# ratan-lab/indelMINER

Hardware: AMD Instinct MI355X
Metric: reads/sec through split-read realign+cluster; VCF diff-clean vs reference (higher is better)
Workload: dtype u8/int32; 1 GPU; BASELINE configs[1]: synthetic 1.0 Mb contig per GPU, 100 bp PE reads at 30x, seeded 1-50 bp indels every ~2 kb, BWA-like S/I/D emission; -k 6 -g 0 -s 1000 -n 10 -q 10; pipeline_depth=4, hip_graph=True, parallelism=contig-sharded x1

## Files before the change

### indelminer_amd/csrc/im_capi.hip

```cpp

#include "im_device.hpp"

#include <stdarg.h>
#include <stdio.h>
#include <stdlib.h>
#include <string.h>

#include <algorithm>
#include <vector>
#include <unordered_map>
#include <mutex>
#include <atomic>

struct ContigArray {
    int32_t* data = nullptr;
    int32_t* sums = nullptr;
    int64_t cap = 0, len = -1;
};

struct GenomeArray {
    int32_t* data = nullptr;
    int32_t* sums = nullptr;
    int32_t flank = 0, min_mapq = 0;
};
// ... 16 lines not shown
    size_t pin_bytes = 0;
    hipStream_t copy_stream = nullptr, back_stream = nullptr;
    hipEvent_t ev_in[2] = {nullptr, nullptr}, ev_k[2] = {nullptr, nullptr}, ev_out[2] = {nullptr, nullptr};
    ContigArray depth, span, pair;
    ContigArray clip_r, clip_l;
    std::vector<int64_t> h_asc_off;
    std::vector<int32_t> h_len;
    int64_t ref_total = 0;
    GenomeArray all_depth, all_span, all_pair;
    GenomeArray all_clip_r, all_clip_l;
    im::TailTable tail = {nullptr, nullptr, 0};
    int32_t tail_min_clip = 0, tail_min_mapq = 0;
    im::LinkTable link = {nullptr, nullptr, 0};
    int32_t link_min_mapq = 0;
    uint32_t* med_scratch = nullptr;
    int32_t med_slots = 0;
    bool med_dirty = false;
    bool support_count_attr = false;
    std::mutex gb_mu;
    std::unordered_map<void*, int32_t> gb_layout;
    std::unordered_map<void*, std::pair<int32_t, int32_t>> fg_layout;
    std::vector<int64_t> h_sums_off;
    void* rg_blob = nullptr;
    im::RgTable rg = {nullptr, 0, 0};
    std::mutex any_mu;
    int32_t* any_list = nullptr; int32_t any_list_cap = 0;
    int32_t* any_counters = nullptr;
    int32_t* any_arena = nullptr; size_t any_arena_bytes = 0;
};

namespace {

char g_err[512] = "";

void set_err(im_ctx* ctx, const char* fmt, ...)
{
    va_list ap;
    va_start(ap, fmt);
    char* dst = ctx ? ctx->err : g_err;
    vsnprintf(dst, 512, fmt, ap);
    va_end(ap);
}

#define HIP_TRY(ctx, expr)                                                              \
    do {                                                                                \
        hipError_t e_ = (expr);                                                         \
        if (e_ != hipSuccess) {                                                         \
// ... 241 lines not shown
    ctx->h_sums_off = sums_off;
    HIP_TRY(ctx, hipMalloc((void**)&g.data, (size_t)ctx->ref_total * sizeof(int32_t)));
    if (scanned) HIP_TRY(ctx, hipMalloc((void**)&g.sums, (size_t)(ints + 1) * sizeof(int32_t)));
    HIP_TRY(ctx, hipMemsetAsync(g.data, 0, (size_t)ctx->ref_total * sizeof(int32_t), ctx->stream));
    if (scanned) HIP_TRY(ctx, hipMemsetAsync(g.sums, 0, (size_t)(ints + 1) * sizeof(int32_t), ctx->stream));
    HIP_TRY(ctx, hipStreamSynchronize(ctx->stream));
    if (flank) { g.flank = *flank; g.min_mapq = min_mapq; }
    return IM_OK;
}

int scan_genome_array(im_ctx* ctx, GenomeArray im_ctx::*which, int32_t tid, void* stream)
{
    if (!ctx || !(ctx->*which).data || tid < 0 || tid >= ctx->n_contigs) return IM_E_ARG;
    const GenomeArray& g = ctx->*which;
    HIP_TRY(ctx, hipSetDevice(ctx->device));
    HIP_TRY(ctx, im::launch_depth_scan_tiled(g.data + ctx->h_asc_off[tid], (int64_t)ctx->h_len[tid] + 1, g.sums + ctx->h_sums_off[tid], (hipStream_t)stream));
    return IM_OK;
}

int reset_genome_array(im_ctx* ctx, GenomeArray im_ctx::*which, int32_t tid, void* stream)
{
    if (!ctx || !(ctx->*which).data || tid < 0 || tid >= ctx->n_contigs) return IM_E_ARG;
    HIP_TRY(ctx, hipSetDevice(ctx->device));
    HIP_TRY(ctx, hipMemsetAsync((ctx->*which).data + ctx->h_asc_off[tid], 0, ((size_t)ctx->h_len[tid] + 1) * sizeof(int32_t), (hipStream_t)stream));
    return IM_OK;
}

int query_genome_array(im_ctx* ctx, GenomeArray im_ctx::*which, int32_t tid, int32_t n, const int32_t* beg, const int32_t* end, Reduce what,
                       uint32_t* out, uint32_t* max_out, const ArgMaxSide* argmax = nullptr)
{
    if (!ctx || n < 0 || !(ctx->*which).data || tid < 0 || tid >= ctx->n_contigs) return IM_E_ARG;
    if (n == 0) return IM_OK;
    if (!beg || !end || !out) return IM_E_ARG;
    const GenomeArray& g = ctx->*which;
    const int32_t* sums = g.sums ? g.sums + ctx->h_sums_off[tid] : nullptr;
    return query_array(ctx, n, beg, end, g.data + ctx->h_asc_off[tid], sums, ctx->h_len[tid], what, out, max_out, argmax);
}

im::RefDev ref_dev(const im_ctx* ctx)
{
    im::RefDev ref;
    ref.ascii = ctx->ref_ascii; ref.pk = reinterpret_cast<const uint8_t*>(ctx->ref_pk);
    ref.asc_off = ctx->d_asc_off; ref.pk_off = ctx->d_pk_off; ref.len = ctx->d_len; ref.n_contigs = ctx->n_contigs;
    return ref;
}

}
// ... 212 lines not shown
        bin_start[b] = e;
        for (int32_t i = n - 1; i >= 0; i--) {
            if (bin[i] != b) continue;
            name_off[e] = (int32_t)names.size();
            name_len[e] = (int32_t)strlen(names_in[i]);
            rmax[e] = range_max[i];
            names.insert(names.end(), names_in[i], names_in[i] + name_len[e] + 1);
            e++;
        }
    }
    bin_start[16] = e;
    std::vector<uint8_t> host((size_t)4 * (20 + 3 * (size_t)m) + names.size() + 8, 0);
    memcpy(host.data(), bin_start.data(), 80);
    memcpy(host.data() + 80, name_off.data(), 4 * (size_t)m);
    memcpy(host.data() + 80 + 4 * (size_t)m, name_len.data(), 4 * (size_t)m);
    memcpy(host.data() + 80 + 8 * (size_t)m, rmax.data(), 4 * (size_t)m);
    if (!names.empty()) memcpy(host.data() + 80 + 12 * (size_t)m, names.data(), names.size());
    const size_t total = (host.size() + 3) / 4 * 4;
    host.resize(total, 0);
    if (ctx->rg_blob) { HIP_TRY(ctx, hipFree(ctx->rg_blob)); ctx->rg_blob = nullptr; }
    HIP_TRY(ctx, hipMalloc(&ctx->rg_blob, total + 256));
    HIP_TRY(ctx, hipMemcpy(ctx->rg_blob, host.data(), total, hipMemcpyHostToDevice));
    ctx->rg.blob = (const uint8_t*)ctx->rg_blob; ctx->rg.n = n; ctx->rg.bytes = (int32_t)total;
    return IM_OK;
}

size_t im_dev_triage_scratch_bytes(int32_t n_records) { return im::triage_scratch_bytes(n_records); }

int im_dev_triage_scratch_init(im_ctx* ctx, int32_t n_records, void* scratch, size_t scratch_bytes, void* stream)
{
    if (!ctx || !scratch || scratch_bytes < im::triage_scratch_bytes(n_records)) return IM_E_ARG;
    HIP_TRY(ctx, hipSetDevice(ctx->device));
    size_t zb = 0;
    const size_t off = im::triage_scratch_zero_offset(n_records, &zb);
    HIP_TRY(ctx, hipMemsetAsync((char*)scratch + off, 0, zb, (hipStream_t)stream));
    return IM_OK;
}

int im_dev_triage(im_ctx* ctx, const im_triage_params* tp, const im_dev_records* recs, const im_dev_cands* out,
                  void* scratch, size_t scratch_bytes, void* stream)
{
    if (!ctx || !tp || !recs || !out) return IM_E_ARG;
    if (!ctx->ref_ascii) { set_err(ctx, "im_set_reference has not been called"); return IM_E_ARG; }
    if (!ctx->rg_blob) { set_err(ctx, "im_set_insert_ranges has not been called"); return IM_E_ARG; }
    if (recs->n < 0 || !out->counters || !out->cand_rec) { set_err(ctx, "bad triage arguments"); return IM_E_ARG; }
    if (scratch_bytes < im::triage_scratch_bytes(recs->n)) { set_err(ctx, "triage scratch too small"); return IM_E_ARG; }
// ... 1297 lines not shown
```

### indelminer_amd/csrc/im_depth.hip

```cpp

#include "im_device.hpp"

namespace im {
namespace {

constexpr int kScanBlock = 256;
constexpr int kScanItems = 8;
constexpr int kScanSub = kScanBlock * kScanItems;
constexpr int kScanSubs = kScanTile / kScanSub;
constexpr int kScanWaves = kScanBlock / 64;
static_assert(kScanTile == kScanSub * kScanSubs, "im_device.hpp names the tile for the queries");
constexpr int kScanGroup = 32;
constexpr int kOffItems = 4;

__global__ __launch_bounds__(256) void depth_scatter_kernel(int32_t n_seg, const int32_t* __restrict__ start, const int32_t* __restrict__ len,
                                                           int64_t clen, int64_t lo, int64_t hi, int32_t* __restrict__ diff)
{
    for (int64_t i = blockIdx.x * (int64_t)blockDim.x + threadIdx.x; i < n_seg; i += (int64_t)gridDim.x * blockDim.x) {
        int64_t a = start[i], b = (int64_t)start[i] + len[i];
        if (a < 0) a = 0;
        if (b > clen) b = clen;
        if (a + lo >= b - hi) continue;
        atomicAdd(&diff[a + lo], 1);
        atomicAdd(&diff[b - hi], -1);
// ... 239 lines not shown
        }
        if (lane == 63) {
#pragma unroll
            for (int s = 0; s < kMedSegs; s++) wsum[s * kMedWaves + wave] = x[s];
        }
        __syncthreads();
        const uint32_t want = (uint32_t)((b - a + 1) / 2);
        uint32_t pre = 0;
#pragma unroll
        for (int s = 0; s < kMedSegs; s++) {
            uint32_t front = 0;
#pragma unroll
            for (int k = 0; k < kMedWaves; k++) { if (k == wave) front = pre; pre += wsum[s * kMedWaves + k]; }
            uint32_t acc = front + x[s] - run[s];
            if (acc < want && want <= acc + run[s]) {
                int e = 0;
                for (; e < 3; e++) { acc += c[s][e]; if (acc >= want) break; }
                out[q] = (uint32_t)((s * kMedBlock + tid) * 4 + e);
            }
        }
    }
}

}

int64_t depth_sums_ints(int64_t clen) { const int64_t t = (clen + 1 + kScanTile - 1) / kScanTile; return t + 1 + (t + kScanGroup - 1) / kScanGroup; }

hipError_t launch_depth_scan_tiled(int32_t* depth, int64_t n, int32_t* sums, hipStream_t stream)
{
    if (n <= 0) return hipSuccess;
    const int64_t tiles = (n + kScanTile - 1) / kScanTile;
    hipLaunchKernelGGL(depth_scan_tiled_kernel, dim3((int)tiles), dim3(kScanBlock), 0, stream, depth, n, sums, (int32_t)tiles);
    return hipGetLastError();
}

hipError_t launch_depth_build(int64_t clen, int32_t n_seg, const int32_t* seg_start, const int32_t* seg_len, int32_t lo, int32_t hi,
                              int32_t* data, int32_t* sums, hipStream_t stream)
{
    const int64_t n = clen + 1;
    hipError_t e = hipMemsetAsync(data, 0, (size_t)n * sizeof(int32_t), stream);
    if (e == hipSuccess) e = hipMemsetAsync(sums, 0, (size_t)depth_sums_ints(clen) * sizeof(int32_t), stream);
    if (e != hipSuccess) return e;
    if (n_seg > 0) {
        int64_t b = ((int64_t)n_seg + 255) / 256;
        if (b > 4096) b = 4096;
        hipLaunchKernelGGL(depth_scatter_kernel, dim3((int)b), dim3(256), 0, stream, n_seg, seg_start, seg_len, clen, (int64_t)lo, (int64_t)hi, data);
// ... 38 lines not shown
```

### indelminer_amd/csrc/im_device.hpp

```cpp
#pragma once

#include <hip/hip_runtime.h>
#include <stdint.h>

#include "indelminer_amd.h"

namespace im {

struct RefDev {
    const uint8_t*  ascii;
    const uint8_t*  pk;
    const int64_t*  asc_off;
    const int64_t*  pk_off;
    const int32_t*  len;
    int32_t         n_contigs;
};

constexpr int kShortRead = 255;
constexpr int kMaxWaveGaps = 60;

struct RealignArgs {
    RefDev      ref;
    im_dev_batch batch;
    im_params   P;
    int32_t     keep_slots;
    const int32_t* n_dev;
    int32_t     first;
};

struct RgTable {
    const uint8_t* blob;
    int32_t n;
    int32_t bytes;
};

size_t triage_scratch_bytes(int32_t n_records);
size_t triage_scratch_zero_offset(int32_t n_records, size_t* bytes);
hipError_t launch_triage(const RefDev& ref, const RgTable& rg, int32_t* depth_diff, const im_triage_params& tp,
                         const im_dev_records& recs, const im_dev_cands& out, void* scratch, hipStream_t stream);

hipError_t launch_flush_cut(const int32_t* cls, const int32_t* b1, const int32_t* b2, int32_t* consumed,
                            int32_t a0, int32_t a1, int32_t b0, int32_t b1_end, int32_t marker, int32_t flush_id,
                            uint64_t* cut_word, const int32_t* cand_rec, const int32_t* n_cand_dev, int32_t cand_cap, hipStream_t stream);
hipError_t launch_flush_seq(const im_flush_desc* desc, int32_t n_fl, const int32_t* cls, const int32_t* b1, const int32_t* b2,
                            int32_t* consumed, const int32_t* cand_rec, const int32_t* n_cand_dev, int32_t cand_cap, int32_t pe_base,
                            int32_t pe_count, hipStream_t stream);
size_t groupby_scratch_bytes(int32_t n_slots);
hipError_t launch_groupby_init(int32_t n_slots, void* scratch, hipStream_t stream);
hipError_t launch_groupby(int32_t n_layout, int32_t n_slots, const int32_t* n_cand_dev, const int32_t* cls, const int32_t* b1, const int32_t* b2, const int32_t* consumed,
                          int32_t tie_desc, int32_t* order, int32_t* cl_key, int32_t* cl_first, int32_t* cl_count,
                          int32_t* counts, void* scratch, hipStream_t stream);
size_t flushgroup_scratch_bytes(int32_t n_slots, int32_t n_fl_cap);
hipError_t launch_flushgroup_init(int32_t n_slots, int32_t n_fl_cap, void* scratch, hipStream_t stream);
hipError_t launch_flush_groupby(int32_t n_slots_layout, int32_t n_fl_layout, const im_flush_desc* desc, int32_t n_fl,
                                const int32_t* cls, const int32_t* b1, const int32_t* b2, int32_t* consumed,
                                const int32_t* cand_rec, const int32_t* n_cand_dev, int32_t cand_cap, int32_t pe_base, int32_t pe_count,
                                int32_t tie_desc, int32_t* order, int32_t* cl_key, int32_t* cl_first, int32_t* cl_count, int32_t* counts,
                                void* scratch, hipStream_t stream);

constexpr int kScanTile = 8192;
int64_t depth_sums_ints(int64_t clen);
hipError_t launch_depth_scan_tiled(int32_t* depth, int64_t n, int32_t* sums, hipStream_t stream);
hipError_t launch_depth_build(int64_t clen, int32_t n_seg, const int32_t* seg_start, const int32_t* seg_len, int32_t lo, int32_t hi,
                              int32_t* data, int32_t* sums, hipStream_t stream);
hipError_t launch_depth_query_tiled(int32_t nq, const int32_t* beg, const int32_t* end, const int32_t* depth, const int32_t* sums,
                                    int64_t clen, uint32_t* out, uint32_t* out_max, hipStream_t stream);
int32_t depth_median_slabs(int32_t beg, int32_t end, int64_t clen);
size_t depth_median_scratch_bytes(int32_t slots);
hipError_t launch_depth_median(int32_t nq, int32_t items, const int32_t* beg, const int32_t* end, const int32_t* first, const int32_t* slot,
                               const int32_t* data, const int32_t* sums, int64_t clen, uint32_t* scratch, int32_t slots, int32_t max_blocks,
                               uint32_t* out, hipStream_t stream);

hipError_t launch_pack_reference(const uint8_t* ascii, uint64_t* pk, int64_t n_bases_padded,
                                 hipStream_t stream);
hipError_t launch_realign(const RealignArgs& a, int n_cu, hipStream_t stream);
hipError_t launch_realign_long(const RealignArgs& a, int n_cu, hipStream_t stream);

hipError_t launch_realign_any_pick(const RealignArgs& a, int all, int32_t* list, int32_t* counters, hipStream_t stream);
size_t realign_any_arena_bytes(int32_t max_read, int32_t max_window, uint32_t numgaps, int32_t lane_shift, int32_t n_waves);
hipError_t launch_realign_any(const RealignArgs& a, const int32_t* list, int32_t* counters, int32_t* arena,
                              int32_t max_read, int32_t max_window, int32_t lane_shift, int32_t n_waves, hipStream_t stream);

hipError_t launch_compact_results(const im_read_result* res, int32_t n_cap, const int32_t* n_dev, int32_t* status, int32_t* slot,
                                  im_read_result* compact, int32_t* count, int n_cu, hipStream_t stream);

// ... 68 lines not shown
```

### indelminer_amd/csrc/im_triage.hip

```cpp

#include "im_device.hpp"
#include "im_rg.hpp"

namespace im {
namespace {

constexpr int kTriBlock = 256;
constexpr int kTriGroup = 32;
constexpr int kTriGroupsMax = 2048;

__device__ __forceinline__ uint32_t ld_u16(const uint8_t* p) { uint16_t v; __builtin_memcpy(&v, p, 2); return v; }


__device__ __forceinline__ uint32_t cigar_word(const RecView& r, uint32_t k)
{
    return k == 0u ? r.cig[0] : k == 1u ? r.cig[1] : k == 2u ? r.cig[2] : k == 3u ? r.cig[3] : ld_u32(r.p + r.o_cigar + 4u * k);
}

__device__ __forceinline__ int32_t aux_int(const RecView& r, const AuxWin& w, uint32_t o)
{
    const uint32_t type = rec_byte(r, w, o);
    if (o + 1u >= r.len) return 0;
    const uint32_t b0 = rec_byte(r, w, o + 1);
    switch (type) {
// ... 171 lines not shown
}

struct TriageArgs {
    im_dev_records recs;
    im_dev_cands out;
    im_triage_params tp;
    RefDev ref;
    RgTable rg;
    int32_t* depth_diff;
    uint32_t* info;
    int32_t* rmax;
    uint2* blk;
    uint32_t* blocks_done;
    uint32_t* grp_done;
    unsigned long long* grp;
    uint2* grp_base;
    int32_t group_size;
    uint32_t* seq_at;
    int32_t* chunk_base;
};

__device__ __forceinline__ uint32_t padded4(int32_t l) { return ((uint32_t)l + 3u) & ~3u; }

constexpr int kDepthWin = 4096;

__global__ __launch_bounds__(kTriBlock, 6) void triage_classify_kernel(TriageArgs A)
{
    __shared__ uint32_t s_cnt[kTriBlock / 64], s_bytes[kTriBlock / 64], s_counted[kTriBlock / 64], s_err[kTriBlock / 64];
    __shared__ uint32_t s_aux[kTriBlock][kAuxWin / 4];
    __shared__ uint32_t s_rg[kRgLds / 4];
    __shared__ int32_t s_generic[2];
    __shared__ int32_t s_dd[kDepthWin];
    __shared__ int32_t s_wpos[kTriBlock / 64], s_wtid[kTriBlock / 64];
    __shared__ uint32_t s_fb[kTriBlock];
    const int t = threadIdx.x, lane = t & 63, wave = t >> 6;
    const int64_t i = (int64_t)blockIdx.x * kTriBlock + t;
    if (A.depth_diff) {
        int4* z = reinterpret_cast<int4*>(s_dd);
#pragma unroll
        for (int k = 0; k < kDepthWin / 4 / kTriBlock; k++) z[t + k * kTriBlock] = make_int4(0, 0, 0, 0);
    }

    RecView r; r.ok = false; r.l_seq = 0; r.flag = 0; r.n_cigar = 0; r.tid = -1; r.pos = 0; r.o_cigar = 0; r.o_seq = 0; r.p = A.recs.raw; r.len = 0; r.o_aux = 0;
    s_fb[t] = 0xFFFFFFFFu;
    if (i < A.recs.n) r = view_record(A.recs.raw, A.recs.rec_off[i], A.recs.rec_off[i + 1]);
    const uint32_t sw_lim = reaches_new_readaln(r) ? (uint32_t)r.l_seq : 0u;
    const uint32_t sw_so = sw_lim ? (uint32_t)(r.p - A.recs.raw) + r.o_seq : 0u;
    BaseSweep S;
    sweep_issue(S, A.recs.raw, sw_so, sw_lim, lane);
    if (r.ok) {
#pragma unroll
        for (int k = 0; k < 4; k++) r.cig[k] = ld_u32(r.p + r.o_cigar + 4u * k);
        const uint32_t aux_bytes = r.len - r.o_aux;
#pragma unroll
        for (int k = 0; k < kAuxWin / 4; k++) if (4u * k < aux_bytes) s_aux[t][k] = ld_u32(r.p + r.o_aux + 4u * k);
    }
    sweep_finish(S, A.recs.raw, sw_so, sw_lim, s_fb + 64 * wave, lane);
    const bool piles = A.depth_diff && r.ok && r.tid >= 0 && r.tid < A.ref.n_contigs && !(r.flag & (0x4u | 0x100u | 0x200u | 0x400u));
    if (A.depth_diff) {
        const uint64_t mp = __ballot(piles);
        const int first = mp ? (int)__builtin_ctzll(mp) : 0;
        const int fp = __shfl(r.pos, first), ft = __shfl(r.tid, first);
        if (lane == 0) { s_wpos[wave] = fp < 0 ? 0 : fp; s_wtid[wave] = mp ? ft : -1; }
    }
    const bool rg_lds = A.rg.bytes <= kRgLds;
    if (rg_lds) for (int k = t; 4 * k < A.rg.bytes; k += kTriBlock) s_rg[k] = reinterpret_cast<const uint32_t*>(A.rg.blob)[k];
    __syncthreads();
    const RgView T = rg_view(rg_lds ? reinterpret_cast<const uint8_t*>(s_rg) : A.rg.blob, A.rg.n);
    if (t == 0) {
        int32_t rm = 0;
        const bool ok = rg_lookup(T, [](uint32_t k) { return (uint32_t)("generic"[k]); }, 7u, rm);
        s_generic[0] = ok ? 1 : 0; s_generic[1] = rm;
    }
    __syncthreads();
    int32_t dd_pos = 0, dd_tid = -1;
    if (A.depth_diff) {
#pragma unroll
        for (int wv = kTriBlock / 64 - 1; wv >= 0; wv--) if (s_wtid[wv] >= 0) { dd_tid = s_wtid[wv]; dd_pos = s_wpos[wv]; }
    }

    uint32_t cls = IM_REC_SKIP, bytes = 0;
    bool cand = false;
    if (i < A.recs.n) {
        AuxWin w; w.lds = s_aux[t]; w.o0 = r.o_aux;
        const Verdict v = classify(r, w, A.tp, T, s_generic[0] != 0, s_generic[1], s_fb[t]);
        cls = v.cls;
        cand = cls == IM_REC_CAND_UNMAPPED || cls == IM_REC_CAND_PROPER;
        if (cand) bytes = padded4(r.l_seq);
        A.info[i] = cls | (v.revcomp ? 0x100u : 0u);
        A.rmax[i] = v.range_max;
        if (A.out.rec_class) A.out.rec_class[i] = (uint8_t)cls;
        if (piles) {
            const int64_t base = A.ref.asc_off[r.tid];
            const int64_t clen = A.ref.len[r.tid];
            const bool here = r.tid == dd_tid;
            int64_t x = r.pos;
            for (uint32_t k = 0; k < r.n_cigar; k++) {
                const uint32_t cw = cigar_word(r, k), op = cw & 15u;
                const int64_t len = cw >> 4;
                if (op == 0u || op == 7u || op == 8u) {
                    int64_t a = x < 0 ? 0 : x, b = x + len > clen ? clen : x + len;
                    if (a < b) {
                        const int64_t ra = a - dd_pos, rb = b - dd_pos;
                        if (here && ra >= 0 && ra < kDepthWin) atomicAdd(&s_dd[ra], 1); else atomicAdd(&A.depth_diff[base + a], 1);
                        if (here && rb >= 0 && rb < kDepthWin) atomicAdd(&s_dd[rb], -1); else atomicAdd(&A.depth_diff[base + b], -1);
                    }
                    x += len;
                } else if (op == 2u || op == 3u) x += len;
            }
        }
    }
    const uint64_t mc = __ballot(cand);
    uint32_t wb = bytes;
#pragma unroll
    for (int o = 32; o > 0; o >>= 1) wb += (uint32_t)__shfl_xor((int)wb, o);
    const uint64_t mk = __ballot(cls != IM_REC_SKIP), me = __ballot(cls >= IM_REC_ERR_RG);
    if (lane == 0) { s_cnt[wave] = (uint32_t)__popcll(mc); s_bytes[wave] = wb; s_counted[wave] = (uint32_t)__popcll(mk); s_err[wave] = (uint32_t)__popcll(me); }
    __syncthreads();
    if (A.depth_diff && dd_tid >= 0) {
        int32_t* dst = A.depth_diff + A.ref.asc_off[dd_tid] + dd_pos;
        const int64_t room = (int64_t)A.ref.len[dd_tid] + 1 - dd_pos;
#pragma unroll 4
        for (int k = 0; k < kDepthWin / kTriBlock; k++) {
            const int idx = t + k * kTriBlock;
            const int32_t v = s_dd[idx];
            if (v != 0 && idx < room) atomicAdd(&dst[idx], v);
        }
    }
    __shared__ uint32_t s_role;
    const int32_t n_blocks = (int32_t)gridDim.x;
    const int32_t gsz = A.group_size, g = (int32_t)blockIdx.x / gsz, g_first = g * gsz;
    const int32_t g_n = min(gsz, n_blocks - g_first), n_groups = (n_blocks + gsz - 1) / gsz;
    if (t == 0) {
        uint32_t c = 0, b = 0, k = 0, e = 0;
        for (int wv = 0; wv < kTriBlock / 64; wv++) { c += s_cnt[wv]; b += s_bytes[wv]; k += s_counted[wv]; e += s_err[wv]; }
        unsigned long long seen = atomicExch(reinterpret_cast<unsigned long long*>(&A.blk[blockIdx.x]),
                                             ((unsigned long long)b << 32) | c | (k << 9) | (e << 18));
        asm volatile("" :: "v"(seen));
        s_role = atomicAdd(&A.grp_done[g], 1u) == (uint32_t)g_n - 1u ? 1u : 0u;
    }
    __syncthreads();
    if (!s_role) return;
    if (t < 64) {
        unsigned long long cb = 0, ke = 0;
        for (int32_t j = t; j < g_n; j += 64) {
            const unsigned long long pv = atomicAdd(reinterpret_cast<unsigned long long*>(&A.blk[g_first + j]), 0ull);
            cb += (pv & 0xFFFFFFFF00000000ull) | ((uint32_t)pv & 511u);
            ke += ((unsigned long long)(((uint32_t)pv >> 9) & 511u) << 32) | (((uint32_t)pv >> 18) & 511u);
        }
#pragma unroll
        for (int o = 32; o > 0; o >>= 1) {
            cb += ((unsigned long long)(uint32_t)__shfl_xor((int)(uint32_t)(cb >> 32), o) << 32) | (uint32_t)__shfl_xor((int)(uint32_t)cb, o);
            ke += ((unsigned long long)(uint32_t)__shfl_xor((int)(uint32_t)(ke >> 32), o) << 32) | (uint32_t)__shfl_xor((int)(uint32_t)ke, o);
        }
        if (t == 0) {
            unsigned long long s0 = atomicExch(&A.grp[2 * g], cb), s1 = atomicExch(&A.grp[2 * g + 1], ke);
            asm volatile("" :: "v"(s0), "v"(s1));
            atomicExch(&A.grp_done[g], 0u);
            s_role = atomicAdd(A.blocks_done, 1u) == (uint32_t)n_groups - 1u ? 2u : 0u;
        }
    }
    __syncthreads();
    if (s_role != 2u) return;
    __shared__ uint32_t wc[kTriBlock / 64], wbb[kTriBlock / 64];
    __shared__ uint32_t carry_c, carry_b, s_ke[2];
    const bool fresh = A.tp.restart != 0;
    if (t == 0) {
        carry_c = fresh ? 0u : (uint32_t)A.out.counters[0]; carry_b = fresh ? 0u : (uint32_t)A.out.counters[1];
        A.chunk_base[0] = (int32_t)carry_c;
        s_ke[0] = 0u; s_ke[1] = 0u;
    }
    uint32_t sum_k = 0, sum_e = 0;
    __syncthreads();
    for (int32_t base = 0; base < n_groups; base += kTriBlock) {
        const int32_t j = base + t;
        uint2 v = make_uint2(0u, 0u);
        if (j < n_groups) {
            const unsigned long long cb = atomicAdd(&A.grp[2 * j], 0ull), ke = atomicAdd(&A.grp[2 * j + 1], 0ull);
            v.x = (uint32_t)cb; v.y = (uint32_t)(cb >> 32);
            sum_k += (uint32_t)(ke >> 32); sum_e += (uint32_t)ke;
        }
        uint32_t c = v.x, b = v.y;
#pragma unroll
        for (int o = 1; o < 64; o <<= 1) {
            const uint32_t tc = (uint32_t)__shfl_up((int)c, o), tb = (uint32_t)__shfl_up((int)b, o);
            if (lane >= o) { c += tc; b += tb; }
        }
        if (lane == 63) { wc[wave] = c; wbb[wave] = b; }
        __syncthreads();
        uint32_t oc = 0, ob = 0;
        for (int wv = 0; wv < wave; wv++) { oc += wc[wv]; ob += wbb[wv]; }
        const uint32_t cc = carry_c, cb0 = carry_b;
        if (j < n_groups) A.grp_base[j] = make_uint2(cc + oc + c - v.x, cb0 + ob + b - v.y);
        __syncthreads();
        if (t == kTriBlock - 1) { carry_c = cc + oc + c; carry_b = cb0 + ob + b; }
        __syncthreads();
    }
#pragma unroll
    for (int o = 32; o > 0; o >>= 1) { sum_k += (uint32_t)__shfl_xor((int)sum_k, o); sum_e += (uint32_t)__shfl_xor((int)sum_e, o); }
    if (lane == 0) { atomicAdd(&s_ke[0], sum_k); atomicAdd(&s_ke[1], sum_e); }
    __syncthreads();
    if (t == 0) {
        A.out.counters[0] = (int32_t)carry_c; A.out.counters[1] = (int32_t)carry_b;
        A.out.counters[2] = (fresh ? 0 : A.out.counters[2]) + (int32_t)s_ke[0];
        A.out.counters[3] = (fresh ? 0 : A.out.counters[3]) + (int32_t)s_ke[1];
        if (fresh) A.out.counters[4] = 0;
        *A.blocks_done = 0u;
    }
}

__device__ __forceinline__ uint32_t base_ascii(uint32_t code)
{
    return code == 1u ? 'A' : code == 2u ? 'C' : code == 4u ? 'G' : code == 8u ? 'T' : code == 15u ? 'N' : 0u;
}
__device__ __forceinline__ uint32_t comp_code(uint32_t c) { return ((c & 1u) << 3) | ((c & 2u) << 1) | ((c & 4u) >> 1) | ((c & 8u) >> 3); }

__global__ __launch_bounds__(kTriBlock) void triage_emit_kernel(TriageArgs A)
{
    __shared__ uint32_t s_cnt[kTriBlock / 64], s_bytes[kTriBlock / 64];
    const int t = threadIdx.x, lane = t & 63, wave = t >> 6;
    const int64_t i = (int64_t)blockIdx.x * kTriBlock + t;
    uint32_t info = 0;
    RecView r; r.ok = false; r.l_seq = 0; r.o_seq = 0; r.p = A.recs.raw;
    if (i < A.recs.n) {
        info = A.info[i];
        const uint32_t cls = info & 255u;
        if (cls == IM_REC_CAND_UNMAPPED || cls == IM_REC_CAND_PROPER) {
            r = view_record(A.recs.raw, A.recs.rec_off[i], A.recs.rec_off[i + 1]);
#pragma unroll
            for (int k = 0; k < 4; k++) r.cig[k] = ld_u32(r.p + r.o_cigar + 4u * k);
        }
    }
    const bool cand = r.ok;
    const uint32_t bytes = cand ? padded4(r.l_seq) : 0u;
    const uint64_t mc = __ballot(cand);
    const uint32_t below = (uint32_t)__popcll(mc & ((1ull << lane) - 1ull));
    uint32_t ib = bytes;
#pragma unroll
    for (int o = 1; o < 64; o <<= 1) { const uint32_t tb = (uint32_t)__shfl_up((int)ib, o); if (lane >= o) ib += tb; }
    if (lane == 63) { s_cnt[wave] = (uint32_t)__popcll(mc); s_bytes[wave] = ib; }
    __shared__ uint2 s_base;
    if (t < 64) {
        const int32_t gsz = A.group_size, g = (int32_t)blockIdx.x / gsz, g_first = g * gsz, mine = (int32_t)blockIdx.x - g_first;
        uint32_t fc = 0, fb = 0;
        for (int32_t j = t; j < mine; j += 64) { const uint2 pv = A.blk[g_first + j]; fc += pv.x & 511u; fb += pv.y; }
#pragma unroll
        for (int o = 32; o > 0; o >>= 1) { fc += (uint32_t)__shfl_xor((int)fc, o); fb += (uint32_t)__shfl_xor((int)fb, o); }
        if (t == 0) { const uint2 gb = A.grp_base[g]; s_base = make_uint2(gb.x + fc, gb.y + fb); }
    }
    __syncthreads();
    if (!cand) return;
    uint32_t oc = 0, ob = 0;
    for (int w = 0; w < wave; w++) { oc += s_cnt[w]; ob += s_bytes[w]; }
    const uint2 base = s_base;
    const uint32_t ci = base.x + oc + below;
    const uint32_t bo = base.y + ob + ib - bytes;
    const im_dev_batch& B = A.out.batch;
    if (!(ci < (uint32_t)A.out.cap_cand && (uint64_t)bo + bytes + 16u <= (uint64_t)A.out.cap_bases)) {
        atomicAdd(&A.out.counters[4], 1);
        if (ci < (uint32_t)A.out.cap_cand) {
            const_cast<int64_t*>(B.base_off)[ci] = 0;
            const_cast<int32_t*>(B.read_len)[ci] = 0;
            A.seq_at[ci - (uint32_t)A.chunk_base[0]] = 0u;
        }
        return;
    }
// ... 82 lines not shown
            }
            *reinterpret_cast<uint32_t*>(dst + p0) = word;
        }
        const uint64_t mb = __ballot(bad);
        const uint32_t half = (uint32_t)(mb >> (32 * ((threadIdx.x >> 5) & 1)));
        if (half != 0u && l32 == 0) {
            const int32_t rec = A.out.cand_rec[ci] - A.recs.rec_base;
            if ((A.info[rec] & 255u) < IM_REC_ERR_RG) {
                if (A.out.rec_class) A.out.rec_class[rec] = (uint8_t)IM_REC_ERR_BASE;
                atomicAdd(&A.out.counters[3], 1);
            }
        }
    }
}

}

constexpr size_t kTriFixedZero = 512 + 4 * (size_t)kTriGroupsMax;
constexpr size_t kTriFixed = kTriFixedZero + 16 * (size_t)kTriGroupsMax + 8 * (size_t)kTriGroupsMax;

size_t triage_scratch_bytes(int32_t n_records)
{
    const size_t n = (size_t)(n_records > 0 ? n_records : 1);
    const size_t blocks = (n + kTriBlock - 1) / kTriBlock;
    auto up = [](size_t x) { return (x + 255) / 256 * 256; };
    return up(n * 4) + up(n * 4) + up(blocks * 8) + up(n * 4) + kTriFixed;
}

size_t triage_scratch_zero_offset(int32_t n_records, size_t* bytes)
{
    (void)n_records;
    *bytes = kTriFixedZero;
    return 0;
}

hipError_t launch_triage(const RefDev& ref, const RgTable& rg, int32_t* depth_diff, const im_triage_params& tp,
                         const im_dev_records& recs, const im_dev_cands& out, void* scratch, hipStream_t stream)
{
    if (recs.n <= 0) return hipSuccess;
    const size_t n = (size_t)recs.n;
    const int blocks = (int)((n + kTriBlock - 1) / kTriBlock);
    auto up = [](size_t x) { return (x + 255) / 256 * 256; };
    TriageArgs A;
    A.recs = recs; A.out = out; A.tp = tp; A.ref = ref; A.rg = rg;
    A.depth_diff = tp.want_depth ? depth_diff : nullptr;
    char* s = static_cast<char*>(scratch);
    A.chunk_base = reinterpret_cast<int32_t*>(s); s += 256;
    A.blocks_done = reinterpret_cast<uint32_t*>(s); s += 256;
    A.grp_done = reinterpret_cast<uint32_t*>(s); s += 4 * (size_t)kTriGroupsMax;
    A.grp = reinterpret_cast<unsigned long long*>(s); s += 16 * (size_t)kTriGroupsMax;
    A.grp_base = reinterpret_cast<uint2*>(s); s += 8 * (size_t)kTriGroupsMax;
    A.group_size = kTriGroup;
    while ((blocks + A.group_size - 1) / A.group_size > kTriGroupsMax) A.group_size *= 2;
    A.info = reinterpret_cast<uint32_t*>(s); s += up(n * 4);
    A.rmax = reinterpret_cast<int32_t*>(s); s += up(n * 4);
    A.blk = reinterpret_cast<uint2*>(s); s += up((size_t)blocks * 8);
    A.seq_at = reinterpret_cast<uint32_t*>(s);
    hipLaunchKernelGGL(triage_classify_kernel, dim3(blocks), dim3(kTriBlock), 0, stream, A);
    hipLaunchKernelGGL(triage_emit_kernel, dim3(blocks), dim3(kTriBlock), 0, stream, A);
    int dgrid = (int)((n + 63) / 64);
    if (dgrid > 16384) dgrid = 16384;
    hipLaunchKernelGGL(triage_decode_kernel, dim3(dgrid), dim3(256), 0, stream, A);
    return hipGetLastError();
}

}
```

Baseline: 5.922 billion reads/s.

## Shrink triage classify to single-wave blocks that fit beside realign waves

The triage classify kernel now runs as 64-lane single-wave workgroups with a smaller LDS footprint (1024-entry depth window, smaller RG table), so it can co-schedule in the LDS left free by concurrent realign waves. Block-wide __syncthreads and shared reductions become wave-level shuffles and fences. The generic read-group lookup moves to host setup, and the grp_done counters are spread across cache lines. The final group scan prefetches eight chunks at a time, the emit kernel maps its group indexing onto the finer classify blocks, and a vectorized fill kernel replaces the per-contig hipMemsetAsync. The cost is many more workgroups and more depth-diff atomics from the narrower window.

```diff
diff --git a/indelminer_amd/csrc/im_capi.hip b/indelminer_amd/csrc/im_capi.hip
--- a/indelminer_amd/csrc/im_capi.hip
+++ b/indelminer_amd/csrc/im_capi.hip
@@ -62,7 +62,7 @@
     std::unordered_map<void*, std::pair<int32_t, int32_t>> fg_layout;
     std::vector<int64_t> h_sums_off;
     void* rg_blob = nullptr;
-    im::RgTable rg = {nullptr, 0, 0};
+    im::RgTable rg = {nullptr, 0, 0, 0, 0};
     std::mutex any_mu;
     int32_t* any_list = nullptr; int32_t any_list_cap = 0;
     int32_t* any_counters = nullptr;
@@ -350,7 +350,7 @@
 {
     if (!ctx || !(ctx->*which).data || tid < 0 || tid >= ctx->n_contigs) return IM_E_ARG;
     HIP_TRY(ctx, hipSetDevice(ctx->device));
-    HIP_TRY(ctx, hipMemsetAsync((ctx->*which).data + ctx->h_asc_off[tid], 0, ((size_t)ctx->h_len[tid] + 1) * sizeof(int32_t), (hipStream_t)stream));
+    HIP_TRY(ctx, im::launch_fill_zero((ctx->*which).data + ctx->h_asc_off[tid], (int64_t)ctx->h_len[tid] + 1, (hipStream_t)stream));
     return IM_OK;
 }
 
@@ -609,6 +609,15 @@
     HIP_TRY(ctx, hipMalloc(&ctx->rg_blob, total + 256));
     HIP_TRY(ctx, hipMemcpy(ctx->rg_blob, host.data(), total, hipMemcpyHostToDevice));
     ctx->rg.blob = (const uint8_t*)ctx->rg_blob; ctx->rg.n = n; ctx->rg.bytes = (int32_t)total;
+    {
+        const char* gname = "generic";
+        uint32_t h = 5381u;
+        for (int k = 6; k >= 0; k--) h += (h << 5) + (uint32_t)(int)gname[k];
+        const int gb = (int)(h & 15u);
+        ctx->rg.generic_ok = 0; ctx->rg.generic_range = 0;
+        for (int32_t k = bin_start[gb]; k < bin_start[gb + 1]; k++)
+            if (name_len[k] >= 7 && memcmp(names.data() + name_off[k], gname, 7) == 0) { ctx->rg.generic_ok = 1; ctx->rg.generic_range = rmax[k]; }
+    }
     return IM_OK;
 }
 
diff --git a/indelminer_amd/csrc/im_depth.hip b/indelminer_amd/csrc/im_depth.hip
--- a/indelminer_amd/csrc/im_depth.hip
+++ b/indelminer_amd/csrc/im_depth.hip
@@ -285,6 +285,27 @@
     }
 }
 
+constexpr int kFillBlock = 256;
+__global__ __launch_bounds__(kFillBlock) void fill_zero_kernel(int32_t* p, int64_t n)
+{
+    const int64_t quads = n / 4;
+    int4* q = reinterpret_cast<int4*>(p);
+    const int64_t stride = (int64_t)gridDim.x * kFillBlock;
+    for (int64_t k = (int64_t)blockIdx.x * kFillBlock + threadIdx.x; k < quads; k += stride) q[k] = make_int4(0, 0, 0, 0);
+    if (blockIdx.x == 0 && 4 * quads + threadIdx.x < n) p[4 * quads + threadIdx.x] = 0;
+}
+
+}
+
+hipError_t launch_fill_zero(int32_t* p, int64_t n, hipStream_t stream)
+{
+    if (n <= 0) return hipSuccess;
+    if (reinterpret_cast<uintptr_t>(p) & 15u) return hipErrorInvalidValue;
+    int64_t b = (n / 4 + 4 * kFillBlock - 1) / (4 * kFillBlock);
+    if (b < 1) b = 1;
+    if (b > 2048) b = 2048;
+    hipLaunchKernelGGL(fill_zero_kernel, dim3((int)b), dim3(kFillBlock), 0, stream, p, n);
+    return hipGetLastError();
 }
 
 int64_t depth_sums_ints(int64_t clen) { const int64_t t = (clen + 1 + kScanTile - 1) / kScanTile; return t + 1 + (t + kScanGroup - 1) / kScanGroup; }
diff --git a/indelminer_amd/csrc/im_device.hpp b/indelminer_amd/csrc/im_device.hpp
--- a/indelminer_amd/csrc/im_device.hpp
+++ b/indelminer_amd/csrc/im_device.hpp
@@ -32,6 +32,7 @@
     const uint8_t* blob;
     int32_t n;
     int32_t bytes;
+    int32_t generic_ok, generic_range;
 };
 
 size_t triage_scratch_bytes(int32_t n_records);
@@ -61,6 +62,7 @@
 constexpr int kScanTile = 8192;
 int64_t depth_sums_ints(int64_t clen);
 hipError_t launch_depth_scan_tiled(int32_t* depth, int64_t n, int32_t* sums, hipStream_t stream);
+hipError_t launch_fill_zero(int32_t* p, int64_t n, hipStream_t stream);
 hipError_t launch_depth_build(int64_t clen, int32_t n_seg, const int32_t* seg_start, const int32_t* seg_len, int32_t lo, int32_t hi,
                               int32_t* data, int32_t* sums, hipStream_t stream);
 hipError_t launch_depth_query_tiled(int32_t nq, const int32_t* beg, const int32_t* end, const int32_t* depth, const int32_t* sums,
diff --git a/indelminer_amd/csrc/im_triage.hip b/indelminer_amd/csrc/im_triage.hip
--- a/indelminer_amd/csrc/im_triage.hip
+++ b/indelminer_amd/csrc/im_triage.hip
@@ -217,27 +217,36 @@
 
 __device__ __forceinline__ uint32_t padded4(int32_t l) { return ((uint32_t)l + 3u) & ~3u; }
 
-constexpr int kDepthWin = 4096;
-
-__global__ __launch_bounds__(kTriBlock, 6) void triage_classify_kernel(TriageArgs A)
-{
-    __shared__ uint32_t s_cnt[kTriBlock / 64], s_bytes[kTriBlock / 64], s_counted[kTriBlock / 64], s_err[kTriBlock / 64];
-    __shared__ uint32_t s_aux[kTriBlock][kAuxWin / 4];
-    __shared__ uint32_t s_rg[kRgLds / 4];
-    __shared__ int32_t s_generic[2];
+constexpr int kClsBlock = 64;
+constexpr int kClsLdsBudget = 6400;
+constexpr int kDepthWin = 1024;
+constexpr int kClsRgLds = 448;
+static_assert(kTriBlock % kClsBlock == 0 && kTriGroup % (kTriBlock / kClsBlock) == 0, "an emit workgroup's classify blocks lie in one group");
+static_assert(kClsBlock * kAuxWin + kClsBlock * 4 + kDepthWin * 4 + kClsRgLds <= kClsLdsBudget, "classify must fit the hole a realign wave leaves");
+
+static_assert(kTriGroupsMax == 64 * 32, "grp_done_slot: 64 lines of 32 words");
+__device__ __forceinline__ int32_t grp_done_slot(int32_t g) { return (g & 63) * 32 + (g >> 6); }
+
+__device__ __forceinline__ void wave_lds_order() { __builtin_amdgcn_fence(__ATOMIC_ACQ_REL, "wavefront"); }
+
+__global__ __launch_bounds__(kClsBlock, 6) void triage_classify_kernel(TriageArgs A)
+{
+    __shared__ uint32_t s_aux[kClsBlock][kAuxWin / 4];
+    __shared__ uint32_t s_rg[kClsRgLds / 4];
     __shared__ int32_t s_dd[kDepthWin];
-    __shared__ int32_t s_wpos[kTriBlock / 64], s_wtid[kTriBlock / 64];
-    __shared__ uint32_t s_fb[kTriBlock];
-    const int t = threadIdx.x, lane = t & 63, wave = t >> 6;
-    const int64_t i = (int64_t)blockIdx.x * kTriBlock + t;
+    __shared__ uint32_t s_fb[kClsBlock];
+    const int lane = threadIdx.x;
+    const int64_t i = (int64_t)blockIdx.x * kClsBlock + lane;
     if (A.depth_diff) {
         int4* z = reinterpret_cast<int4*>(s_dd);
 #pragma unroll
-        for (int k = 0; k < kDepthWin / 4 / kTriBlock; k++) z[t + k * kTriBlock] = make_int4(0, 0, 0, 0);
+        for (int k = 0; k < kDepthWin / 4 / kClsBlock; k++) z[lane + k * kClsBlock] = make_int4(0, 0, 0, 0);
     }
 
     RecView r; r.ok = false; r.l_seq = 0; r.flag = 0; r.n_cigar = 0; r.tid = -1; r.pos = 0; r.o_cigar = 0; r.o_seq = 0; r.p = A.recs.raw; r.len = 0; r.o_aux = 0;
-    s_fb[t] = 0xFFFFFFFFu;
+    s_fb[lane] = 0xFFFFFFFFu;
+    const bool rg_lds = A.rg.bytes <= kClsRgLds;
+    if (rg_lds) for (int k = lane; 4 * k < A.rg.bytes; k += kClsBlock) s_rg[k] = reinterpret_cast<const uint32_t*>(A.rg.blob)[k];
     if (i < A.recs.n) r = view_record(A.recs.raw, A.recs.rec_off[i], A.recs.rec_off[i + 1]);
     const uint32_t sw_lim = reaches_new_readaln(r) ? (uint32_t)r.l_seq : 0u;
     const uint32_t sw_so = sw_lim ? (uint32_t)(r.p - A.recs.raw) + r.o_seq : 0u;
@@ -248,37 +257,26 @@
         for (int k = 0; k < 4; k++) r.cig[k] = ld_u32(r.p + r.o_cigar + 4u * k);
         const uint32_t aux_bytes = r.len - r.o_aux;
 #pragma unroll
-        for (int k = 0; k < kAuxWin / 4; k++) if (4u * k < aux_bytes) s_aux[t][k] = ld_u32(r.p + r.o_aux + 4u * k);
-    }
-    sweep_finish(S, A.recs.raw, sw_so, sw_lim, s_fb + 64 * wave, lane);
+        for (int k = 0; k < kAuxWin / 4; k++) if (4u * k < aux_bytes) s_aux[lane][k] = ld_u32(r.p + r.o_aux + 4u * k);
+    }
+    wave_lds_order();
+    sweep_finish(S, A.recs.raw, sw_so, sw_lim, s_fb, lane);
     const bool piles = A.depth_diff && r.ok && r.tid >= 0 && r.tid < A.ref.n_contigs && !(r.flag & (0x4u | 0x100u | 0x200u | 0x400u));
+    int32_t dd_pos = 0, dd_tid = -1;
     if (A.depth_diff) {
         const uint64_t mp = __ballot(piles);
         const int first = mp ? (int)__builtin_ctzll(mp) : 0;
         const int fp = __shfl(r.pos, first), ft = __shfl(r.tid, first);
-        if (lane == 0) { s_wpos[wave] = fp < 0 ? 0 : fp; s_wtid[wave] = mp ? ft : -1; }
-    }
-    const bool rg_lds = A.rg.bytes <= kRgLds;
-    if (rg_lds) for (int k = t; 4 * k < A.rg.bytes; k += kTriBlock) s_rg[k] = reinterpret_cast<const uint32_t*>(A.rg.blob)[k];
-    __syncthreads();
+        dd_pos = fp < 0 ? 0 : fp; dd_tid = mp ? ft : -1;
+    }
+    wave_lds_order();
     const RgView T = rg_view(rg_lds ? reinterpret_cast<const uint8_t*>(s_rg) : A.rg.blob, A.rg.n);
-    if (t == 0) {
-        int32_t rm = 0;
-        const bool ok = rg_lookup(T, [](uint32_t k) { return (uint32_t)("generic"[k]); }, 7u, rm);
-        s_generic[0] = ok ? 1 : 0; s_generic[1] = rm;
-    }
-    __syncthreads();
-    int32_t dd_pos = 0, dd_tid = -1;
-    if (A.depth_diff) {
-#pragma unroll
-        for (int wv = kTriBlock / 64 - 1; wv >= 0; wv--) if (s_wtid[wv] >= 0) { dd_tid = s_wtid[wv]; dd_pos = s_wpos[wv]; }
-    }
 
     uint32_t cls = IM_REC_SKIP, bytes = 0;
     bool cand = false;
     if (i < A.recs.n) {
-        AuxWin w; w.lds = s_aux[t]; w.o0 = r.o_aux;
-        const Verdict v = classify(r, w, A.tp, T, s_generic[0] != 0, s_generic[1], s_fb[t]);
+        AuxWin w; w.lds = s_aux[lane]; w.o0 = r.o_aux;
+        const Verdict v = classify(r, w, A.tp, T, A.rg.generic_ok != 0, A.rg.generic_range, s_fb[lane]);
         cls = v.cls;
         cand = cls == IM_REC_CAND_UNMAPPED || cls == IM_REC_CAND_PROPER;
         if (cand) bytes = padded4(r.l_seq);
@@ -310,35 +308,32 @@
 #pragma unroll
     for (int o = 32; o > 0; o >>= 1) wb += (uint32_t)__shfl_xor((int)wb, o);
     const uint64_t mk = __ballot(cls != IM_REC_SKIP), me = __ballot(cls >= IM_REC_ERR_RG);
-    if (lane == 0) { s_cnt[wave] = (uint32_t)__popcll(mc); s_bytes[wave] = wb; s_counted[wave] = (uint32_t)__popcll(mk); s_err[wave] = (uint32_t)__popcll(me); }
-    __syncthreads();
+    wave_lds_order();
     if (A.depth_diff && dd_tid >= 0) {
         int32_t* dst = A.depth_diff + A.ref.asc_off[dd_tid] + dd_pos;
         const int64_t room = (int64_t)A.ref.len[dd_tid] + 1 - dd_pos;
 #pragma unroll 4
-        for (int k = 0; k < kDepthWin / kTriBlock; k++) {
-            const int idx = t + k * kTriBlock;
+        for (int k = 0; k < kDepthWin / kClsBlock; k++) {
+            const int idx = lane + k * kClsBlock;
             const int32_t v = s_dd[idx];
             if (v != 0 && idx < room) atomicAdd(&dst[idx], v);
         }
     }
-    __shared__ uint32_t s_role;
     const int32_t n_blocks = (int32_t)gridDim.x;
     const int32_t gsz = A.group_size, g = (int32_t)blockIdx.x / gsz, g_first = g * gsz;
     const int32_t g_n = min(gsz, n_blocks - g_first), n_groups = (n_blocks + gsz - 1) / gsz;
-    if (t == 0) {
-        uint32_t c = 0, b = 0, k = 0, e = 0;
-        for (int wv = 0; wv < kTriBlock / 64; wv++) { c += s_cnt[wv]; b += s_bytes[wv]; k += s_counted[wv]; e += s_err[wv]; }
+    uint32_t role = 0;
+    if (lane == 0) {
         unsigned long long seen = atomicExch(reinterpret_cast<unsigned long long*>(&A.blk[blockIdx.x]),
-                                             ((unsigned long long)b << 32) | c | (k << 9) | (e << 18));
+                                             ((unsigned long long)wb << 32) | (uint32_t)__popcll(mc) | ((uint32_t)__popcll(mk) << 9) | ((uint32_t)__popcll(me) << 18));
         asm volatile("" :: "v"(seen));
-        s_role = atomicAdd(&A.grp_done[g], 1u) == (uint32_t)g_n - 1u ? 1u : 0u;
-    }
-    __syncthreads();
-    if (!s_role) return;
-    if (t < 64) {
+        role = atomicAdd(&A.grp_done[grp_done_slot(g)], 1u) == (uint32_t)g_n - 1u ? 1u : 0u;
+    }
+    role = (uint32_t)__shfl((int)role, 0);
+    if (!role) return;
+    {
         unsigned long long cb = 0, ke = 0;
-        for (int32_t j = t; j < g_n; j += 64) {
+        for (int32_t j = lane; j < g_n; j += 64) {
             const unsigned long long pv = atomicAdd(reinterpret_cast<unsigned long long*>(&A.blk[g_first + j]), 0ull);
             cb += (pv & 0xFFFFFFFF00000000ull) | ((uint32_t)pv & 511u);
             ke += ((unsigned long long)(((uint32_t)pv >> 9) & 511u) << 32) | (((uint32_t)pv >> 18) & 511u);
@@ -348,57 +343,50 @@
             cb += ((unsigned long long)(uint32_t)__shfl_xor((int)(uint32_t)(cb >> 32), o) << 32) | (uint32_t)__shfl_xor((int)(uint32_t)cb, o);
             ke += ((unsigned long long)(uint32_t)__shfl_xor((int)(uint32_t)(ke >> 32), o) << 32) | (uint32_t)__shfl_xor((int)(uint32_t)ke, o);
         }
-        if (t == 0) {
+        role = 0;
+        if (lane == 0) {
             unsigned long long s0 = atomicExch(&A.grp[2 * g], cb), s1 = atomicExch(&A.grp[2 * g + 1], ke);
             asm volatile("" :: "v"(s0), "v"(s1));
-            atomicExch(&A.grp_done[g], 0u);
-            s_role = atomicAdd(A.blocks_done, 1u) == (uint32_t)n_groups - 1u ? 2u : 0u;
-        }
-    }
-    __syncthreads();
-    if (s_role != 2u) return;
-    __shared__ uint32_t wc[kTriBlock / 64], wbb[kTriBlock / 64];
-    __shared__ uint32_t carry_c, carry_b, s_ke[2];
+            atomicExch(&A.grp_done[grp_done_slot(g)], 0u);
+            role = atomicAdd(A.blocks_done, 1u) == (uint32_t)n_groups - 1u ? 2u : 0u;
+        }
+        role = (uint32_t)__shfl((int)role, 0);
+    }
+    if (role != 2u) return;
     const bool fresh = A.tp.restart != 0;
-    if (t == 0) {
-        carry_c = fresh ? 0u : (uint32_t)A.out.counters[0]; carry_b = fresh ? 0u : (uint32_t)A.out.counters[1];
-        A.chunk_base[0] = (int32_t)carry_c;
-        s_ke[0] = 0u; s_ke[1] = 0u;
-    }
+    uint32_t carry_c = fresh ? 0u : (uint32_t)A.out.counters[0], carry_b = fresh ? 0u : (uint32_t)A.out.counters[1];
+    if (lane == 0) A.chunk_base[0] = (int32_t)carry_c;
     uint32_t sum_k = 0, sum_e = 0;
-    __syncthreads();
-    for (int32_t base = 0; base < n_groups; base += kTriBlock) {
-        const int32_t j = base + t;
-        uint2 v = make_uint2(0u, 0u);
-        if (j < n_groups) {
-            const unsigned long long cb = atomicAdd(&A.grp[2 * j], 0ull), ke = atomicAdd(&A.grp[2 * j + 1], 0ull);
-            v.x = (uint32_t)cb; v.y = (uint32_t)(cb >> 32);
-            sum_k += (uint32_t)(ke >> 32); sum_e += (uint32_t)ke;
-        }
-        uint32_t c = v.x, b = v.y;
-#pragma unroll
-        for (int o = 1; o < 64; o <<= 1) {
-            const uint32_t tc = (uint32_t)__shfl_up((int)c, o), tb = (uint32_t)__shfl_up((int)b, o);
-            if (lane >= o) { c += tc; b += tb; }
-        }
-        if (lane == 63) { wc[wave] = c; wbb[wave] = b; }
-        __syncthreads();
-        uint32_t oc = 0, ob = 0;
-        for (int wv = 0; wv < wave; wv++) { oc += wc[wv]; ob += wbb[wv]; }
-        const uint32_t cc = carry_c, cb0 = carry_b;
-        if (j < n_groups) A.grp_base[j] = make_uint2(cc + oc + c - v.x, cb0 + ob + b - v.y);
-        __syncthreads();
-        if (t == kTriBlock - 1) { carry_c = cc + oc + c; carry_b = cb0 + ob + b; }
-        __syncthreads();
+    constexpr int kAhead = 8;
+    for (int32_t base = 0; base < n_groups; base += kAhead * 64) {
+        unsigned long long cbv[kAhead], kev[kAhead];
+#pragma unroll
+        for (int q = 0; q < kAhead; q++) {
+            const int32_t j = base + 64 * q + lane;
+            cbv[q] = 0ull; kev[q] = 0ull;
+            if (j < n_groups) { cbv[q] = atomicAdd(&A.grp[2 * j], 0ull); kev[q] = atomicAdd(&A.grp[2 * j + 1], 0ull); }
+        }
+#pragma unroll
+        for (int q = 0; q < kAhead; q++) {
+            const int32_t j = base + 64 * q + lane;
+            const uint32_t vx = (uint32_t)cbv[q], vy = (uint32_t)(cbv[q] >> 32);
+            sum_k += (uint32_t)(kev[q] >> 32); sum_e += (uint32_t)kev[q];
+            uint32_t c = vx, b = vy;
+#pragma unroll
+            for (int o = 1; o < 64; o <<= 1) {
+                const uint32_t tc = (uint32_t)__shfl_up((int)c, o), tb = (uint32_t)__shfl_up((int)b, o);
+                if (lane >= o) { c += tc; b += tb; }
+            }
+            if (j < n_groups) A.grp_base[j] = make_uint2(carry_c + c - vx, carry_b + b - vy);
+            carry_c += (uint32_t)__shfl((int)c, 63); carry_b += (uint32_t)__shfl((int)b, 63);
+        }
     }
 #pragma unroll
     for (int o = 32; o > 0; o >>= 1) { sum_k += (uint32_t)__shfl_xor((int)sum_k, o); sum_e += (uint32_t)__shfl_xor((int)sum_e, o); }
-    if (lane == 0) { atomicAdd(&s_ke[0], sum_k); atomicAdd(&s_ke[1], sum_e); }
-    __syncthreads();
-    if (t == 0) {
+    if (lane == 0) {
         A.out.counters[0] = (int32_t)carry_c; A.out.counters[1] = (int32_t)carry_b;
-        A.out.counters[2] = (fresh ? 0 : A.out.counters[2]) + (int32_t)s_ke[0];
-        A.out.counters[3] = (fresh ? 0 : A.out.counters[3]) + (int32_t)s_ke[1];
+        A.out.counters[2] = (fresh ? 0 : A.out.counters[2]) + (int32_t)sum_k;
+        A.out.counters[3] = (fresh ? 0 : A.out.counters[3]) + (int32_t)sum_e;
         if (fresh) A.out.counters[4] = 0;
         *A.blocks_done = 0u;
     }
@@ -436,7 +424,8 @@
     if (lane == 63) { s_cnt[wave] = (uint32_t)__popcll(mc); s_bytes[wave] = ib; }
     __shared__ uint2 s_base;
     if (t < 64) {
-        const int32_t gsz = A.group_size, g = (int32_t)blockIdx.x / gsz, g_first = g * gsz, mine = (int32_t)blockIdx.x - g_first;
+        const int32_t mine0 = (int32_t)blockIdx.x * (kTriBlock / kClsBlock);
+        const int32_t gsz = A.group_size, g = mine0 / gsz, g_first = g * gsz, mine = mine0 - g_first;
         uint32_t fc = 0, fb = 0;
         for (int32_t j = t; j < mine; j += 64) { const uint2 pv = A.blk[g_first + j]; fc += pv.x & 511u; fb += pv.y; }
 #pragma unroll
@@ -565,7 +554,7 @@
 size_t triage_scratch_bytes(int32_t n_records)
 {
     const size_t n = (size_t)(n_records > 0 ? n_records : 1);
-    const size_t blocks = (n + kTriBlock - 1) / kTriBlock;
+    const size_t blocks = (n + kClsBlock - 1) / kClsBlock;
     auto up = [](size_t x) { return (x + 255) / 256 * 256; };
     return up(n * 4) + up(n * 4) + up(blocks * 8) + up(n * 4) + kTriFixed;
 }
@@ -582,7 +571,7 @@
 {
     if (recs.n <= 0) return hipSuccess;
     const size_t n = (size_t)recs.n;
-    const int blocks = (int)((n + kTriBlock - 1) / kTriBlock);
+    const int blocks = (int)((n + kTriBlock - 1) / kTriBlock), cls_blocks = (int)((n + kClsBlock - 1) / kClsBlock);
     auto up = [](size_t x) { return (x + 255) / 256 * 256; };
     TriageArgs A;
     A.recs = recs; A.out = out; A.tp = tp; A.ref = ref; A.rg = rg;
@@ -594,12 +583,12 @@
     A.grp = reinterpret_cast<unsigned long long*>(s); s += 16 * (size_t)kTriGroupsMax;
     A.grp_base = reinterpret_cast<uint2*>(s); s += 8 * (size_t)kTriGroupsMax;
     A.group_size = kTriGroup;
-    while ((blocks + A.group_size - 1) / A.group_size > kTriGroupsMax) A.group_size *= 2;
+    while ((cls_blocks + A.group_size - 1) / A.group_size > kTriGroupsMax) A.group_size *= 2;
     A.info = reinterpret_cast<uint32_t*>(s); s += up(n * 4);
     A.rmax = reinterpret_cast<int32_t*>(s); s += up(n * 4);
-    A.blk = reinterpret_cast<uint2*>(s); s += up((size_t)blocks * 8);
+    A.blk = reinterpret_cast<uint2*>(s); s += up((size_t)cls_blocks * 8);
     A.seq_at = reinterpret_cast<uint32_t*>(s);
-    hipLaunchKernelGGL(triage_classify_kernel, dim3(blocks), dim3(kTriBlock), 0, stream, A);
+    hipLaunchKernelGGL(triage_classify_kernel, dim3(cls_blocks), dim3(kClsBlock), 0, stream, A);
     hipLaunchKernelGGL(triage_emit_kernel, dim3(blocks), dim3(kTriBlock), 0, stream, A);
     int dgrid = (int)((n + 63) / 64);
     if (dgrid > 16384) dgrid = 16384;
diff --git a/profiles/dispatch_overlap.py b/profiles/dispatch_overlap.py
--- /dev/null
+++ b/profiles/dispatch_overlap.py
@@ -0,0 +1,92 @@
+#!/usr/bin/env python3
+import bisect
+import csv
+import glob
+import os
+import sys
+
+BUCKETS = [(0.0, 0.05), (0.05, 0.25), (0.25, 0.5), (0.5, 0.75), (0.75, 0.95), (0.95, 1.0001)]
+
+
+def load(d):
+    paths = [d] if os.path.isfile(d) else sorted(glob.glob(os.path.join(d, "**", "*kernel_trace.csv"), recursive=True))
+    rows = []
+    for p in paths:
+        with open(p, newline="") as f:
+            for r in csv.DictReader(f):
+                rows.append((r["Kernel_Name"], r.get("Queue_Id", "0"), int(r["Start_Timestamp"]), int(r["End_Timestamp"])))
+    rows.sort(key=lambda r: r[2])
+    return rows
+
+
+def union(iv):
+    out = []
+    for s, e in sorted(iv):
+        if out and s <= out[-1][1]:
+            out[-1][1] = max(out[-1][1], e)
+        else:
+            out.append([s, e])
+    return out
+
+
+def covered(u, starts, s, e):
+    k = max(bisect.bisect_right(starts, s) - 1, 0)
+    tot = 0
+    while k < len(u) and u[k][0] < e:
+        tot += max(0, min(e, u[k][1]) - max(s, u[k][0]))
+        k += 1
+    return tot
+
+
+def beside(rows, mine, other, out):
+    queues = sorted({q for _, q, _, _ in rows})
+    per_q = {}
+    for q in queues:
+        u = union([(s, e) for n, qq, s, e in rows if other in n and qq != q])
+        per_q[q] = (u, [x[0] for x in u])
+    got = []
+    for n, q, s, e in rows:
+        if mine in n and e > s:
+            u, st = per_q[q]
+            got.append((covered(u, st, s, e) / (e - s), (e - s) / 1e3))
+    out.append("%s: %d dispatches, mean %.1f us; run time inside a %s dispatch of another queue: mean share %.2f"
+               % (mine, len(got), sum(d for _, d in got) / max(len(got), 1), other, sum(f for f, _ in got) / max(len(got), 1)))
+    out.append("  share inside      dispatches   mean us   median us")
+    for lo, hi in BUCKETS:
+        ds = sorted(d for f, d in got if lo <= f < hi)
+        if ds:
+            out.append("  %.2f - %.2f       %8d   %7.1f   %7.1f" % (lo, min(hi, 1.0), len(ds), sum(ds) / len(ds), ds[len(ds) // 2]))
+    return got
+
+
+def main():
+    d = sys.argv[1]
+    tag = sys.argv[2] if len(sys.argv) > 2 else ""
+    rows = load(d)
+    cut = len(rows) // 10
+    rows = rows[cut:len(rows) - cut]
+    out = ["%s %d dispatches in the window, %.1f ms" % (tag, len(rows), (rows[-1][3] - rows[0][2]) / 1e6)]
+    n_step = sum(1 for n, _, _, _ in rows if "triage_classify_kernel" in n)
+    out.append("classify dispatches (= steps) %d: %.1f us of wall time per step under the tracer" % (n_step, (rows[-1][3] - rows[0][2]) / 1e3 / max(n_step, 1)))
+    beside(rows, "triage_classify_kernel", "realign_kernel", out)
+    beside(rows, "realign_kernel", "triage_classify_kernel", out)
+    tot = {}
+    for n, _, s, e in rows:
+        k = n.replace("(anonymous namespace)::", "").replace("void ", "").split("(")[0]
+        tot[k] = tot.get(k, 0) + (e - s)
+    out.append("kernel time per step, us:")
+    for k, v in sorted(tot.items(), key=lambda kv: -kv[1]):
+        out.append("  %-60s %7.1f" % (k[:60], v / 1e3 / max(n_step, 1)))
+    out.append("idle between consecutive dispatches of one queue:")
+    for q in sorted({q for _, q, _, _ in rows}):
+        mine = [(s, e) for _, qq, s, e in rows if qq == q]
+        gaps = sorted(max(0, mine[k + 1][0] - mine[k][1]) / 1e3 for k in range(len(mine) - 1))
+        if gaps:
+            span = (mine[-1][1] - mine[0][0]) / 1e3
+            out.append("  queue %s: %d dispatches, idle %.1f %% of its span; gap mean %.2f us, median %.2f, 90th percentile %.2f"
+                       % (q, len(mine), 100.0 * sum(gaps) / span, sum(gaps) / len(gaps), gaps[len(gaps) // 2], gaps[len(gaps) * 9 // 10]))
+    print("\n".join(out))
+
+
+if __name__ == "__main__":
+    main()
diff --git a/profiles/launch_rate_probe.hip b/profiles/launch_rate_probe.hip
--- /dev/null
+++ b/profiles/launch_rate_probe.hip
@@ -0,0 +1,36 @@
+#include <hip/hip_runtime.h>
+#include <cstdio>
+
+#define TRY(x) do { hipError_t e_ = (x); if (e_ != hipSuccess) { fprintf(stderr, "%s: %s\n", #x, hipGetErrorString(e_)); return 1; } } while (0)
+
+__global__ void empty_kernel(int* out)
+{
+    extern __shared__ int lds[];
+    lds[threadIdx.x] = (int)blockIdx.x;
+    if (out) out[0] = lds[threadIdx.x ^ 1];
+}
+
+int main()
+{
+    hipStream_t st; TRY(hipStreamCreate(&st));
+    hipEvent_t a, b; TRY(hipEventCreate(&a)); TRY(hipEventCreate(&b));
+    const int grids[] = { 1172, 4688, 12232, 73153 };
+    const int shapes[][2] = { { 64, 256 }, { 64, 6400 }, { 64, 25756 }, { 256, 1024 }, { 256, 25756 } };
+    printf("lanes  lds_B   grid   us_per_launch  ns_per_workgroup\n");
+    for (auto& sh : shapes) {
+        TRY(hipFuncSetAttribute(reinterpret_cast<const void*>(empty_kernel), hipFuncAttributeMaxDynamicSharedMemorySize, sh[1]));
+        for (int g : grids) {
+            float best = 1e30f;
+            for (int rep = 0; rep < 20; rep++) {
+                TRY(hipEventRecord(a, st));
+                hipLaunchKernelGGL(empty_kernel, dim3(g), dim3(sh[0]), sh[1], st, nullptr);
+                TRY(hipEventRecord(b, st));
+                TRY(hipEventSynchronize(b));
+                float ms = 0; TRY(hipEventElapsedTime(&ms, a, b));
+                if (ms < best) best = ms;
+            }
+            printf("%5d  %5d  %5d  %13.1f  %16.2f\n", sh[0], sh[1], g, best * 1e3f, best * 1e6f / g);
+        }
+    }
+    return 0;
+}
```

New measurement: 6.481 billion reads/s, median of 6. 1.09x the previous value.
